# trinh-hoang-hiep/Collaborative-Filtering-Kafka

Measured on AMD Instinct MI355X. Metric: ALS ratings/sec per full iteration, k=64 Netflix-shape, 1/2/4/8 MI355X, higher is better.
Workload: dtype f32; 1 GPU; netflix-shape synthetic 480189 users x 17770 movies x 100000000 ratings, k=64, lambda=0.05, one step = one full ALS iteration; workload_name=netflix, n_movies=17770, nnz=100000000, nnz_this_rank=100000000, k=64, seed=2581, partitions=1, parallelism=id%1 shards + RCCL all-gather, rccl_world=1, exchange_world=1, rehearsal_gloo_one_gpu=False

## Files before the change

collaborative-filtering-kafka_amd/csrc/als_engine.cpp:

```cpp
#include <hip/hip_runtime.h>
#include <rccl/rccl.h>

#include <algorithm>
#include <chrono>
#include <cstdarg>
#include <cstdio>
#include <cstdlib>
#include <cstring>
#include <string>
#include <thread>
#include <vector>

#include "als.h"
#include "als_internal.h"

using cfk::Path;
using cfk::Task;

namespace {

thread_local std::string g_last_error;

int fail(int code, const char* fmt, ...) {
    char buf[1024];
// ... 8 lines not shown
#define HIP_TRY(expr)                                                                              \
    do {                                                                                           \
        hipError_t _e = (expr);                                                                    \
        if (_e != hipSuccess)                                                                      \
            return fail(ALS_ERR_DEVICE, "%s failed: %s (%s:%d)", #expr, hipGetErrorString(_e),     \
                        __FILE__, __LINE__);                                                       \
    } while (0)

struct Block {
    bool set = false;
    int64_t n_rows = 0, row_offset = 0, n_opp_rows = 0, nnz = 0, nnz_padded = 0;
    int32_t* d_col = nullptr;
    float* d_rat = nullptr;
    uint32_t* d_rat_pk = nullptr;
    int32_t* d_col_ps = nullptr;
    Task* d_tasks = nullptr;
    Task* d_reduce = nullptr;
    int32_t n_tasks = 0, n_reduce = 0, n_slots = 0;
    double* d_task_se = nullptr;
    std::vector<Task> h_tasks, h_reduce;
    Task* d_ctasks = nullptr;
    Task* d_creduce = nullptr;
    std::vector<int32_t> coff, croff;
    Task* d_dual[3] = {nullptr, nullptr, nullptr};
    int32_t n_dual[3] = {0, 0, 0};
    std::vector<Task> h_dual[3];
    Task* d_cdual[3] = {nullptr, nullptr, nullptr};
    std::vector<int32_t> cdoff[3];
    Task* d_sq_tasks = nullptr;
    int32_t n_sq = 0;
    cfk::BlockLayout layout;
    int64_t ilv_rows = 0, ilv_tasks = 0;
    int64_t rows_per_chunk = 0, chunk_stride = 0;
    int64_t factor_row(int64_t i) const {
        return rows_per_chunk > 0 ? row_offset + (i / rows_per_chunk) * chunk_stride + i % rows_per_chunk
                                  : row_offset + i;
    }
};

struct TimingRec {
    int side;
    hipEvent_t ev[3];
};

struct Factors {
    void* ptr = nullptr;
    int64_t n_rows = 0;
    bool owned = false;
};

struct Settings {
    cfk::PlanKnobs plan;
    bool gram_f32 = false;
    bool force_valu = false;
    float refine_min_pivot = 0.45f;
    bool dual_side = true;
    int64_t comm_timeout_ms = 120000;
    int32_t debug_flags = 0;
    uint32_t debug_gen_skew = 0;
    int32_t debug_extra_lds = 0;
    bool debug_fixed_gen = false;
};

}

namespace cfk_detail {
void set_last_error(const std::string& s) { g_last_error = s; }
}

struct als_engine {
    int device = 0;
    int k = 0, kp = 0;
    int precision = ALS_F32;
    Path path = Path::VALU;
    hipStream_t stream = nullptr;
    bool own_stream = false;
    Block blk[2];
    Factors fac[2];
    void* d_partials = nullptr;
    size_t partial_bytes = 0;
    int64_t generic_slabs = 0;
    void* d_split = nullptr;
    size_t split_bytes = 0;
    uint32_t* d_amax = nullptr;
    void* d_rec = nullptr;
    size_t rec_bytes = 0;
    void* h_stage = nullptr;
    size_t stage_bytes = 0;
    uint32_t* d_integrity = nullptr;
    int cu_count = 0;
    Settings cfg;
    uint32_t gen = 0;
    ncclComm_t comm = nullptr;
    int world = 1, rank = 0;
    hipStream_t comm_stream = nullptr;
    hipEvent_t solved = nullptr;
    hipEvent_t gathered[2] = {nullptr, nullptr};
    bool gather_pending[2] = {false, false};
    int last_gather_side = -1;
    int64_t last_gather_chunk = -1, last_gather_rows = 0;
    hipStream_t side_stream = nullptr;
    hipEvent_t fork = nullptr, join = nullptr;
    bool timing = false;
    std::vector<hipEvent_t> ev_pool;
    std::vector<TimingRec> pending;
    size_t elem() const { return precision == ALS_F64 ? 8 : 4; }
};

namespace {

int check_engine(const als_engine* e) {
    if (!e) return fail(ALS_ERR_INVALID_ARGUMENT, "engine is NULL");
    return ALS_OK;
}

int wait_gathers(als_engine* e, bool movie, bool user) {
    const bool want[2] = {movie, user};
    for (int s = 0; s < 2; ++s)
        if (want[s] && e->gather_pending[s]) {
            HIP_TRY(hipStreamWaitEvent(e->stream, e->gathered[s], 0));
            e->gather_pending[s] = false;
        }
    return ALS_OK;
}

int stream_wait(als_engine* e, hipStream_t s) {
    if (!e->comm || e->cfg.comm_timeout_ms <= 0) {
        HIP_TRY(hipStreamSynchronize(s));
        return ALS_OK;
    }
    const auto t0 = std::chrono::steady_clock::now();
    for (int spin = 0;; ++spin) {
        const hipError_t st = hipStreamQuery(s);
        if (st == hipSuccess) return ALS_OK;
        if (st != hipErrorNotReady) return fail(ALS_ERR_DEVICE, "stream wait: %s", hipGetErrorString(st));
        const int64_t ms =
            std::chrono::duration_cast<std::chrono::milliseconds>(std::chrono::steady_clock::now() - t0).count();
        if (ms > e->cfg.comm_timeout_ms) {
            (void)ncclCommAbort(e->comm);
            e->comm = nullptr;
            return fail(ALS_ERR_COMM,
                        "rank %d of %d: the engine's stream did not complete within %lld ms; the last RCCL all-gather "
                        "issued was side %s chunk %lld (%lld rows per shard); communicator aborted",
                        e->rank, e->world, (long long)e->cfg.comm_timeout_ms,
                        e->last_gather_side == ALS_SIDE_MOVIE ? "movie" : e->last_gather_side == ALS_SIDE_USER ? "user"
                                                                                                              : "none",
                        (long long)e->last_gather_chunk, (long long)e->last_gather_rows);
        }
        if (spin < 1000) std::this_thread::yield();
        else std::this_thread::sleep_for(std::chrono::microseconds(50));
    }
}

int sync_checked(als_engine* e) {
    if (int r = wait_gathers(e, true, true)) return r;
    if (int r = stream_wait(e, e->stream)) return r;
    uint32_t rec[cfk::INTEGRITY_WORDS];
    HIP_TRY(hipMemcpy(rec, e->d_integrity, sizeof(rec), hipMemcpyDeviceToHost));
    if (rec[0] != 0)
        return fail(ALS_ERR_INTEGRITY,
                    "%u REDUCE tasks found partial slots that failed their check (first: launch generation %u, slot "
                    "%u, row %u): partial sums its PARTIAL task's writes had not reached",
                    rec[0], rec[1], rec[2], rec[3]);
    return ALS_OK;
}
int check_side(int side) {
    if (side != ALS_SIDE_MOVIE && side != ALS_SIDE_USER)
// ... 36 lines not shown
#endif
    }
    if (const char* env = getenv("ALS_COMM_TIMEOUT_S")) c.comm_timeout_ms = (int64_t)(atof(env) * 1000.0);
#ifdef CFK_DEBUG_KNOBS
    if (const char* env = getenv("ALS_DEBUG_SKIP_SOLVE"))
        if (env[0] == '1') c.debug_flags |= cfk::SOLVE_FLAG_SKIP_SOLVE;
    if (const char* env = getenv("ALS_DEBUG_SKIP_REFINE"))
        if (env[0] == '1') c.debug_flags |= cfk::SOLVE_FLAG_SKIP_REFINE;
    if (const char* env = getenv("ALS_DEBUG_REDUCE_GEN_SKEW")) c.debug_gen_skew = (uint32_t)atoi(env);
    if (const char* env = getenv("ALS_DEBUG_FIXED_GEN")) c.debug_fixed_gen = env[0] == '1';
    if (const char* env = getenv("ALS_DEBUG_EXTRA_LDS")) c.debug_extra_lds = atoi(env);
    if (const char* env = getenv("ALS_ILV_CHUNK")) c.plan.ilv_chunk = std::max(32L, atol(env));
    if (const char* env = getenv("ALS_TASK_ORDER")) {
        if (std::strncmp(env, "stagger", 7) == 0) {
            c.plan.task_order = cfk::PlanKnobs::STAGGER;
            if (env[7] == ':') c.plan.stagger_window = std::max(1, atoi(env + 8));
        }
        if (std::strcmp(env, "random") == 0) c.plan.task_order = cfk::PlanKnobs::RANDOM;
    }
#endif
    return c;
}
}

extern "C" {

int als_abi_version(void) { return ALS_ABI_VERSION; }

int als_device_count(int* n) {
    if (!n) return fail(ALS_ERR_INVALID_ARGUMENT, "n is NULL");
    *n = 0;
    HIP_TRY(hipGetDeviceCount(n));
    return ALS_OK;
}
const char* als_last_error(void) { return g_last_error.c_str(); }

#define CFK_STR2(x) #x
#define CFK_STR(x) CFK_STR2(x)
const char* als_build_source_sha256(void) {
#ifdef CFK_SOURCE_SHA256
    return &CFK_STR(CFK_SOURCE_SHA256)[1];
#else
    return "";
#endif
}

int als_engine_create(int device, int num_features, int precision, als_engine** out) {
    if (!out) return fail(ALS_ERR_INVALID_ARGUMENT, "out is NULL");
    *out = nullptr;
    if (precision != ALS_F32 && precision != ALS_F64)
        return fail(ALS_ERR_INVALID_ARGUMENT, "precision must be ALS_F32 or ALS_F64");
    if (num_features < 1) return fail(ALS_ERR_INVALID_ARGUMENT, "num_features must be >= 1, got %d", num_features);
    if (num_features > 1024)
        return fail(ALS_ERR_UNSUPPORTED, "num_features=%d: this build supports 1..1024", num_features);
    const bool generic = num_features > (precision == ALS_F64 ? 64 : 128);
    int kp = num_features <= 16 ? 16 : num_features <= 32 ? 32 : num_features <= 64 ? 64 : 128;
    if (generic) kp = (num_features + 15) / 16 * 16;
    Path path = generic ? Path::GENERIC : (precision == ALS_F32 && num_features >= 32) ? Path::MFMA_SPLIT : Path::VALU;
    const Settings cfg = read_environment();
    if (path == Path::MFMA_SPLIT && cfg.gram_f32) path = Path::MFMA;
    if (cfg.force_valu && !generic) path = Path::VALU;
    if (!cfk::variant_available(precision, kp, path))
        return fail(ALS_ERR_UNSUPPORTED, "no kernel variant for precision=%d kp=%d", precision, kp);
    int ndev = 0;
    HIP_TRY(hipGetDeviceCount(&ndev));
    if (device < 0 || device >= ndev) return fail(ALS_ERR_INVALID_ARGUMENT, "device %d out of range (%d devices)", device, ndev);
    HIP_TRY(hipSetDevice(device));
    als_engine* e = new als_engine();
    e->device = device;
    e->k = num_features;
    e->kp = kp;
    e->precision = precision;
    e->path = path;
    e->cfg = cfg;
    hipError_t st = hipStreamCreateWithFlags(&e->stream, hipStreamNonBlocking);
    if (st != hipSuccess) {
        delete e;
        return fail(ALS_ERR_DEVICE, "hipStreamCreate: %s", hipGetErrorString(st));
    }
    e->own_stream = true;
    st = hipDeviceGetAttribute(&e->cu_count, hipDeviceAttributeMultiprocessorCount, device);
    if (st == hipSuccess) st = hipMalloc((void**)&e->d_integrity, cfk::INTEGRITY_WORDS * sizeof(uint32_t));
    if (st == hipSuccess) st = hipMemset(e->d_integrity, 0, cfk::INTEGRITY_WORDS * sizeof(uint32_t));
    if (st == hipSuccess) st = hipMalloc((void**)&e->d_amax, 2 * sizeof(uint32_t));
    if (st != hipSuccess) {
        (void)hipStreamDestroy(e->stream);
        (void)hipFree(e->d_integrity);
        (void)hipFree(e->d_amax);
        delete e;
        return fail(ALS_ERR_DEVICE, "integrity record: %s", hipGetErrorString(st));
    }
    *out = e;
    return ALS_OK;
}

int als_engine_destroy(als_engine* e) {
    if (!e) return ALS_OK;
    (void)hipSetDevice(e->device);
    (void)hipStreamSynchronize(e->stream);
    for (auto& b : e->blk) free_block(b);
    for (auto& f : e->fac)
        if (f.owned) (void)hipFree(f.ptr);
    (void)hipFree(e->d_partials);
    (void)hipFree(e->d_split);
    (void)hipFree(e->d_rec);
    (void)hipHostFree(e->h_stage);
    (void)hipFree(e->d_integrity);
    (void)hipFree(e->d_amax);
    for (auto& rec : e->pending)
        for (auto ev : rec.ev) (void)hipEventDestroy(ev);
    for (auto ev : e->ev_pool) (void)hipEventDestroy(ev);
    if (e->comm_stream) (void)hipStreamSynchronize(e->comm_stream);
    if (e->comm) (void)ncclCommDestroy(e->comm);
    if (e->comm_stream) (void)hipStreamDestroy(e->comm_stream);
    for (auto ev : {e->solved, e->gathered[0], e->gathered[1]})
        if (ev) (void)hipEventDestroy(ev);
    if (e->side_stream) {
        (void)hipStreamSynchronize(e->side_stream);
        (void)hipStreamDestroy(e->side_stream);
    }
    for (auto ev : {e->fork, e->join})
        if (ev) (void)hipEventDestroy(ev);
    if (e->own_stream) (void)hipStreamDestroy(e->stream);
    delete e;
    return ALS_OK;
}

int als_engine_set_stream(als_engine* e, void* hip_stream) {
    if (int r = check_engine(e)) return r;
    HIP_TRY(hipSetDevice(e->device));
    if (e->own_stream) {
        HIP_TRY(hipStreamSynchronize(e->stream));
        HIP_TRY(hipStreamDestroy(e->stream));
        e->own_stream = false;
        e->stream = nullptr;
    }
    if (hip_stream) {
        e->stream = (hipStream_t)hip_stream;
    } else {
        HIP_TRY(hipStreamCreateWithFlags(&e->stream, hipStreamNonBlocking));
        e->own_stream = true;
    }
    return ALS_OK;
}

int als_engine_use_default_stream(als_engine* e) {
    if (int r = check_engine(e)) return r;
    HIP_TRY(hipSetDevice(e->device));
    if (e->own_stream) {
        HIP_TRY(hipStreamSynchronize(e->stream));
        HIP_TRY(hipStreamDestroy(e->stream));
        e->own_stream = false;
    }
    e->stream = nullptr;
    return ALS_OK;
}

int als_factor_stride(const als_engine* e) { return e ? e->kp : 0; }

}

namespace {

int ensure_stage(als_engine* e) {
    constexpr size_t STAGE = 32u << 20;
    if (!e->h_stage) {
        HIP_TRY(hipHostMalloc(&e->h_stage, STAGE, hipHostMallocDefault));
        e->stage_bytes = STAGE;
    }
    return ALS_OK;
}

int check_block_shape(als_engine* e, int64_t n_rows, int64_t row_offset, int64_t n_opp_rows) {
    if (n_rows < 0 || row_offset < 0 || n_opp_rows < 0)
        return fail(ALS_ERR_INVALID_ARGUMENT, "negative size (n_rows=%lld row_offset=%lld n_opp_rows=%lld)",
                    (long long)n_rows, (long long)row_offset, (long long)n_opp_rows);
    if (n_rows > INT32_MAX) return fail(ALS_ERR_UNSUPPORTED, "n_rows exceeds 2^31-1");
    if (n_opp_rows >= INT32_MAX) return fail(ALS_ERR_UNSUPPORTED, "n_opp_rows must be < 2^31-1 (int32 column indices)");
    if ((n_opp_rows + 1) * (int64_t)e->kp * (int64_t)e->elem() > (int64_t)UINT32_MAX)
        return fail(ALS_ERR_UNSUPPORTED, "opposite factor matrix exceeds 4 GiB (32-bit gather offsets)");
    return ALS_OK;
}

inline int64_t padded(int64_t d) { return (d + cfk::BLOCK_ENTRIES - 1) / cfk::BLOCK_ENTRIES * cfk::BLOCK_ENTRIES; }

int upload_tasks(Task** dst, const std::vector<Task>& src) {
    if (*dst) {
        (void)hipFree(*dst);
        *dst = nullptr;
    }
    const size_t bytes = src.size() * sizeof(Task);
// ... 290 lines not shown
    const size_t row_bytes = (size_t)e->kp * es;
    if (int r = ensure_stage(e)) return r;
    const int64_t rows_per = (int64_t)(e->stage_bytes / row_bytes);
    for (int64_t r = 0; r < n_rows; r += rows_per) {
        const int64_t nr = std::min(rows_per, n_rows - r);
        HIP_TRY(cfk::launch_download((const char*)f.ptr + (size_t)(row0 + r) * row_bytes, e->h_stage,
                                     (size_t)nr * row_bytes, e->stream));
        HIP_TRY(hipStreamSynchronize(e->stream));
        const char* stage = (const char*)e->h_stage;
        char* dst = (char*)host_dst + (size_t)r * dst_ld * es;
        for (int64_t i = 0; i < nr; ++i)
            std::memcpy(dst + (size_t)i * dst_ld * es, stage + i * row_bytes, (size_t)e->k * es);
    }
    return ALS_OK;
}

namespace {

struct DualLaunch {
    const Task* t[3] = {nullptr, nullptr, nullptr};
    int32_t n[3] = {0, 0, 0};
};

int launch_half(als_engine* e, int side, float lambda, const Task* tasks, int32_t n_tasks, const Task* reduce,
                int32_t n_reduce, bool first_chunk, const DualLaunch& dl) {
    Block& b = e->blk[side];
    const Factors& self = e->fac[side];
    const Factors& opp = e->fac[1 - side];
    if (!self.ptr || !opp.ptr) return fail(ALS_ERR_STATE, "als_solve_half: factor matrices not allocated/bound");
    if (b.n_rows > 0 && b.factor_row(b.n_rows - 1) >= self.n_rows)
        return fail(ALS_ERR_STATE, "block rows (last at factor row %lld) exceed factor rows %lld",
                    (long long)b.factor_row(b.n_rows - 1), (long long)self.n_rows);
    if (b.n_opp_rows != opp.n_rows)
        return fail(ALS_ERR_STATE, "block was set for %lld opposite rows, the opposite factor matrix has %lld",
                    (long long)b.n_opp_rows, (long long)opp.n_rows);
    if (!(lambda >= 0.f)) return fail(ALS_ERR_INVALID_ARGUMENT, "lambda must be >= 0");
    HIP_TRY(hipSetDevice(e->device));
    if (int r = wait_gathers(e, side == ALS_SIDE_USER || first_chunk, side == ALS_SIDE_MOVIE || first_chunk)) return r;
    cfk::SolveArgs a{};
    a.tasks = tasks;
    a.n_tasks = n_tasks;
    a.k = e->k;
    a.col = b.d_col;
    a.rat = b.d_rat;
    a.opp = opp.ptr;
    a.out = self.ptr;
    a.row_offset = b.row_offset;
    a.rows_per_chunk = (int32_t)b.rows_per_chunk;
    a.chunk_stride = b.chunk_stride;
    a.partials = e->d_partials;
    a.scratch_slabs = e->generic_slabs;
    a.lambda = lambda;
    a.sentinel = (int32_t)b.n_opp_rows;
    a.flags = e->path == Path::VALU ? 0 : e->cfg.debug_flags;
    if (++e->gen == 0) e->gen = 1;
    a.gen = e->cfg.debug_fixed_gen ? 1u : e->gen;
    a.integrity = e->d_integrity;
    a.refine_min_pivot = e->cfg.refine_min_pivot;
    a.extra_lds = e->cfg.debug_extra_lds;
    TimingRec rec{side, {nullptr, nullptr, nullptr}};
    if (e->timing) {
        for (auto& ev : rec.ev) {
            if (!e->ev_pool.empty()) {
                ev = e->ev_pool.back();
                e->ev_pool.pop_back();
            } else {
                HIP_TRY(hipEventCreate(&ev));
            }
        }
        HIP_TRY(hipEventRecord(rec.ev[0], e->stream));
    }
    const bool any_dual = dl.n[0] > 0 || dl.n[1] > 0 || dl.n[2] > 0;
    const bool side_dual = any_dual && e->cfg.dual_side;
    if (side_dual) {
        if (!e->side_stream) {
            HIP_TRY(hipStreamCreateWithFlags(&e->side_stream, hipStreamNonBlocking));
            HIP_TRY(hipEventCreateWithFlags(&e->fork, hipEventDisableTiming));
            HIP_TRY(hipEventCreateWithFlags(&e->join, hipEventDisableTiming));
        }
        HIP_TRY(hipEventRecord(e->fork, e->stream));
    }
    if (b.layout.presplit) {
        if (first_chunk) {
            const int64_t n_floats = (b.n_opp_rows + 1) * (int64_t)e->kp;
            HIP_TRY(cfk::launch_absmax((const float*)opp.ptr, n_floats, e->kp, e->d_amax, e->stream));
            HIP_TRY(cfk::launch_presplit(e->kp, (const float*)opp.ptr, e->d_split, b.n_opp_rows + 1, e->d_amax,
                                         e->stream));
        }
        a.opp_split = e->d_split;
        a.rat_pk = b.d_rat_pk;
        a.rat_lo_off = b.nnz_padded / 2;
        a.col_ps = b.d_col_ps;
        a.amax = e->d_amax;
    }
    HIP_TRY(cfk::launch_solve(e->precision, e->kp, e->path, a, e->stream, b.layout.presplit, false));
    if (b.layout.presplit) {
        cfk::SolveArgs f = a;
        f.presplit_fallback = 1;
        f.grid_cap = 4 * e->cu_count;
        HIP_TRY(cfk::launch_solve(e->precision, e->kp, e->path, f, e->stream, false, false));
    }
    if (side_dual) HIP_TRY(hipStreamWaitEvent(e->side_stream, e->fork, 0));
    for (int c = 0; c < 3; ++c)
        if (dl.n[c] > 0) {
            cfk::SolveArgs d = a;
            d.tasks = dl.t[c];
            d.n_tasks = dl.n[c];
            HIP_TRY(cfk::launch_dual(e->kp, 2 * (c + 1), d, side_dual ? e->side_stream : e->stream));
        }
    if (side_dual) {
        HIP_TRY(hipEventRecord(e->join, e->side_stream));
        HIP_TRY(hipStreamWaitEvent(e->stream, e->join, 0));
    }
    if (e->timing) HIP_TRY(hipEventRecord(rec.ev[1], e->stream));
    if (n_reduce > 0) {
        a.tasks = reduce;
        a.n_tasks = n_reduce;
        a.gen += e->cfg.debug_gen_skew;
        HIP_TRY(cfk::launch_solve(e->precision, e->kp, e->path, a, e->stream, false, true));
    }
    if (e->timing) {
        HIP_TRY(hipEventRecord(rec.ev[2], e->stream));
        e->pending.push_back(rec);
    }
    return ALS_OK;
}

}

int als_solve_half(als_engine* e, int side, float lambda) {
    if (int r = check_engine(e)) return r;
    if (int r = check_side(side)) return r;
    Block& b = e->blk[side];
    if (!b.set) return fail(ALS_ERR_STATE, "als_solve_half: no block set for side %d", side);
    DualLaunch dl;
    for (int c = 0; c < 3; ++c) {
        dl.t[c] = b.d_dual[c];
        dl.n[c] = b.n_dual[c];
    }
    return launch_half(e, side, lambda, b.d_tasks, b.n_tasks, b.d_reduce, b.n_reduce, true, dl);
}

int als_set_chunks(als_engine* e, int side, int n_chunks, const int64_t* row_bounds) {
    if (int r = check_engine(e)) return r;
    if (int r = check_side(side)) return r;
    Block& b = e->blk[side];
    if (!b.set) return fail(ALS_ERR_STATE, "als_set_chunks: no block set for side %d", side);
    if (n_chunks < 1 || !row_bounds) return fail(ALS_ERR_INVALID_ARGUMENT, "n_chunks must be >= 1 with row_bounds");
    if (row_bounds[0] != 0 || row_bounds[n_chunks] != b.n_rows)
        return fail(ALS_ERR_INVALID_ARGUMENT, "row_bounds must run from 0 to n_rows (%lld)", (long long)b.n_rows);
    for (int c = 0; c < n_chunks; ++c)
        if (row_bounds[c + 1] < row_bounds[c]) return fail(ALS_ERR_INVALID_ARGUMENT, "row_bounds not monotone");
    std::vector<Task> ct, cr, cdl[3];
    cfk::partition_by_chunk(b.h_tasks, n_chunks, row_bounds, ct, b.coff);
    cfk::partition_by_chunk(b.h_reduce, n_chunks, row_bounds, cr, b.croff);
    for (int c = 0; c < 3; ++c) cfk::partition_by_chunk(b.h_dual[c], n_chunks, row_bounds, cdl[c], b.cdoff[c]);
    HIP_TRY(hipSetDevice(e->device));
    HIP_TRY(hipStreamSynchronize(e->stream));
    if (int r = upload_tasks(&b.d_ctasks, ct)) return r;
    if (int r = upload_tasks(&b.d_creduce, cr)) return r;
    for (int c = 0; c < 3; ++c)
        if (int r = upload_tasks(&b.d_cdual[c], cdl[c])) return r;
    return ALS_OK;
}

int als_solve_half_chunk(als_engine* e, int side, float lambda, int chunk) {
    if (int r = check_engine(e)) return r;
    if (int r = check_side(side)) return r;
    Block& b = e->blk[side];
    if (!b.set || b.coff.empty()) return fail(ALS_ERR_STATE, "als_solve_half_chunk: no chunks set for side %d", side);
    if (chunk < 0 || chunk + 1 >= (int)b.coff.size())
        return fail(ALS_ERR_INVALID_ARGUMENT, "chunk %d out of range (%d chunks)", chunk, (int)b.coff.size() - 1);
    DualLaunch dl;
    for (int c = 0; c < 3; ++c) {
        dl.t[c] = b.d_cdual[c] + b.cdoff[c][chunk];
        dl.n[c] = b.cdoff[c][chunk + 1] - b.cdoff[c][chunk];
// ... 438 lines not shown
```

collaborative-filtering-kafka_amd/csrc/als_internal.h:

```cpp
#pragma once
#include <cstdint>
#include <string>
#include <vector>

#include <hip/hip_runtime.h>

#include "als_plan.h"

namespace cfk {

struct SolveArgs {
    const Task* tasks;
    int32_t n_tasks;
    int32_t k;
    const int32_t* col;
    const float* rat;
    const void* opp;
    void* out;
    int64_t row_offset;
    void* partials;
    float lambda;
    int32_t sentinel;
    int32_t flags;
    const void* opp_split;
    uint32_t gen;
    uint32_t* integrity;
    float refine_min_pivot;
    const uint32_t* rat_pk;
    const int32_t* col_ps;
    int32_t rows_per_chunk;
    int64_t chunk_stride;
    int64_t rat_lo_off;
    const uint32_t* amax;
    int32_t presplit_fallback;
    int64_t scratch_slabs;
    int32_t grid_cap;
    int32_t extra_lds;
};
__host__ __device__ inline int64_t factor_row(int64_t row_offset, int32_t rows_per_chunk, int64_t chunk_stride,
                                              int32_t row) {
    if (rows_per_chunk <= 0) return row_offset + row;
    const int32_t q = row / rows_per_chunk;
    return row_offset + (int64_t)q * chunk_stride + (row - q * rows_per_chunk);
}
constexpr int INTEGRITY_WORDS = 4;
constexpr int32_t SOLVE_FLAG_SKIP_SOLVE = 1;
constexpr int32_t SOLVE_FLAG_SKIP_REFINE = 2;

struct SqErrArgs {
    const Task* tasks;
    int32_t n_tasks;
    const int32_t* col;
    const float* rat;
    const void* opp;
    const void* self;
    int64_t row_offset;
    double* task_se;
    int32_t sentinel;
    int32_t rows_per_chunk;
    int64_t chunk_stride;
};

struct GenericPlan {
    bool g_in_lds;
    int batch;
    int64_t lds_bytes;
    int64_t slab_elems;
};
GenericPlan generic_plan(int precision, int kp);
hipError_t launch_generic(int precision, int kp, const SolveArgs& a, hipStream_t s);

hipError_t launch_solve(int precision, int kp, Path path, const SolveArgs& a, hipStream_t s, bool presplit,
                        bool reduce);
hipError_t launch_permute_blocks(const int32_t* col, const float* rat, int32_t* col_out, float* rat_out,
                                 const int32_t* perm, int64_t n_blocks, hipStream_t s);
hipError_t launch_dual(int kp, int cd, const SolveArgs& a, hipStream_t s);
hipError_t launch_absmax(const float* src, int64_t n_floats, int kp, uint32_t* amax , hipStream_t s);
hipError_t launch_presplit(int kp, const float* src, void* dst, int64_t n_rows, const uint32_t* amax, hipStream_t s);
hipError_t launch_pack_cols_ps(const int32_t* col, int32_t* dst, int64_t n_entries, hipStream_t s);
hipError_t launch_pack_ratings(const float* rat, uint32_t* dst, int64_t n_pairs, hipStream_t s);
hipError_t launch_upload(const void* host_pinned, void* dst, size_t bytes, hipStream_t s);
hipError_t launch_download(const void* src, void* host_pinned, size_t bytes, hipStream_t s);
hipError_t launch_predict(int precision, const void* U, const void* M, int kp, int k, const int64_t* urows,
                          int64_t n_u, const int64_t* mrows, int64_t n_m, float* out, hipStream_t s);
hipError_t launch_recommend(int precision, const void* U, const void* M, int kp, int k, const int64_t* urows,
                            int64_t n_users, const int64_t* mrows, int64_t n_cand, int top_n,
                            const RecommendPlan& plan, const int64_t* excl_ptr, const int32_t* excl_idx,
                            float* part_score, int32_t* part_pos, float* out_score, int32_t* out_pos, hipStream_t s);
hipError_t launch_sq_error(int precision, int kp, const SqErrArgs& a, hipStream_t s);
int partial_words_per_lane(int precision, int kp, Path path);
int build_block_device(const int32_t* rows, const int32_t* cols, const int16_t* ratings, int64_t nnz, int64_t n_rows,
                       int64_t n_opp_rows, hipStream_t s, std::vector<int64_t>& deg, std::vector<int64_t>& begin,
                       int32_t** d_col, float** d_rat, std::string& err);
bool variant_available(int precision, int kp, Path path);

}
```

collaborative-filtering-kafka_amd/csrc/als_kernels.hip:

```cpp
#include <hip/hip_runtime.h>

#include <mutex>
#include <type_traits>
#include <utility>
#include <vector>

#include "als_internal.h"
#include "als_device.h"
#include "als_slots.h"
#include "als_lds_solve.h"
#include "als_mfma.h"
#include "als_tile_solve.h"
#include "als_gram.h"
#include "als_gram_presplit.h"
#include "als_generic.h"

namespace cfk {
namespace {

template <int KP>
constexpr int mfma_waves() { return WAVES; }

__global__ __launch_bounds__(256) void als_absmax(const u32x4* __restrict__ src, int64_t n4, int vpr,
                                                  uint32_t* __restrict__ out) {
    uint32_t m = 0, rmin = 0xffffffffu;
    const int64_t stride = (int64_t)gridDim.x * 256;
    for (int64_t i0 = (int64_t)blockIdx.x * 256 + (threadIdx.x & ~63); i0 < n4; i0 += stride) {
        const int64_t i = i0 + (threadIdx.x & 63);
        uint32_t v = 0;
        if (i < n4) {
            const u32x4 x = src[i] & 0x7fffffffu;
            v = max(max(x[0], x[1]), max(x[2], x[3]));
        }
        m = max(m, v);
        for (int o = 1; o < vpr; o <<= 1) v = max(v, (uint32_t)__shfl_xor((int)v, o));
        if (v != 0 && i < n4) rmin = min(rmin, v);
    }
#pragma unroll
    for (int o = 32; o > 0; o >>= 1) {
        m = max(m, (uint32_t)__shfl_xor((int)m, o));
        rmin = min(rmin, (uint32_t)__shfl_xor((int)rmin, o));
    }
    __shared__ uint32_t wm[4], wr[4];
    if ((threadIdx.x & 63) == 0) {
        wm[threadIdx.x >> 6] = m;
        wr[threadIdx.x >> 6] = rmin;
    }
    __syncthreads();
    if (threadIdx.x == 0) {
        m = max(max(wm[0], wm[1]), max(wm[2], wm[3]));
        rmin = min(min(wr[0], wr[1]), min(wr[2], wr[3]));
        if (m != 0) atomicMax(out, m);
        if (rmin != 0xffffffffu) atomicMax(out + 1, ~rmin);
    }
}
constexpr float PRESPLIT_RANGE = 65536.f;
__device__ __forceinline__ bool presplit_ok(const uint32_t* st) {
    const uint32_t mx = st[0], rc = st[1];
    if (mx >= 0x7f800000u) return false;
    if (rc == 0) return true;
    return __uint_as_float(mx) <= PRESPLIT_RANGE * __uint_as_float(~rc);
}

template <int KP>
__global__ __launch_bounds__(256) void als_presplit(const float* __restrict__ src, unsigned* __restrict__ dst,
                                                   int64_t n_threads, const uint32_t* __restrict__ amax) {
    constexpr int C = KP / 16;
    const int64_t t = (int64_t)blockIdx.x * 256 + threadIdx.x;
    if (t >= n_threads) return;
    const int sc = split_exp(*amax);
    const int64_t row = t / (2 * C);
    const int b = (int)(t % (2 * C)) >> 1, jh = (int)(t & 1);
    const float* s = src + row * KP + C * 8 * jh + b;
    u32x4 h, m;
#pragma unroll
    for (int i = 0; i < 4; ++i) {
        unsigned hh, mm;
        split2(ldexpf(s[C * (2 * i)], sc), ldexpf(s[C * (2 * i + 1)], sc), hh, mm);
        h[i] = hh;
        m[i] = mm;
    }
    unsigned* o = dst + row * (presplit_row_bytes(KP) / 4) + (16 * b + 8 * jh) / 2;
    *(u32x4*)o = h;
    *(u32x4*)(o + KP / 2) = m;
}
__global__ __launch_bounds__(256) void als_pack_cols_ps(const int32_t* __restrict__ col, int32_t* __restrict__ dst,
                                                       int64_t n) {
    const int64_t i = (int64_t)blockIdx.x * 256 + threadIdx.x;
    if (i >= n) return;
    const int w = (int)(i & 31), r = w >> 2, x = w & 3;
    const int k = 16 * (x >> 1) + 8 * (r >> 2) + 4 * (x & 1) + (r & 3);
    dst[i] = col[(i & ~(int64_t)31) + k];
}

template <int KP, int MINW, bool SPLIT, bool PRESPLIT = false, bool REDUCE = false, bool GRIDLOOP = false>
__global__ __launch_bounds__(64 * mfma_waves<KP>(), MINW) void als_solve_mfma(SolveArgs a) {
    constexpr int C = KP / 16;
    constexpr int NW = mfma_waves<KP>();
    using Acc = MfmaAcc<C>;
    __shared__ __attribute__((aligned(16))) float sbuf[NW][KP];
    constexpr bool TILES_LDS = tiles_in_lds<C>() && !(PRESPLIT && !REDUCE);
    constexpr int TL = TILES_LDS ? tile_lds_floats<C>() : 0;
    __shared__ __attribute__((aligned(16))) float tiles_lds[NW][TL > 0 ? TL : 1];
    (void)tiles_lds;
    constexpr int STAGE = (PRESPLIT && !REDUCE) ? 2 * C * 1024 : 16;
    __shared__ __attribute__((aligned(1024))) unsigned char stage_lds[NW][STAGE];
    (void)stage_lds;

    const int wave = threadIdx.x >> 6, lane = threadIdx.x & 63;
    if constexpr (!REDUCE && SPLIT) {
        if (PRESPLIT ? !presplit_ok(a.amax) : (a.presplit_fallback && presplit_ok(a.amax))) return;
    }
    auto task = [&](const int tid) {
        const Task tk = load_task(a.tasks + tid);
        float* buf = sbuf[wave];

        Acc acc;
#pragma unroll
        for (int p = 0; p < Acc::NT; ++p) acc.g[p] = f32x4{0.f, 0.f, 0.f, 0.f};
#pragma unroll
        for (int c = 0; c < C; ++c) acc.rhs[c] = 0.f;
        f32x4 E[C];
#pragma unroll
        for (int c = 0; c < C; ++c) E[c] = f32x4{0.f, 0.f, 0.f, 0.f};

        int ps_sc = 0;
        if constexpr (REDUCE) sum_partial_slots<C>(a, tk, acc, lane);
        else if constexpr (PRESPLIT) ps_sc = gram_presplit<KP>(a, tk, acc, E, stage_lds[uni(wave)], buf, lane);
        else if constexpr (SPLIT) gram_split<KP>(a, tk, acc, E, lane);
        else gram_f32<KP>(a, tk, acc, lane);

        if constexpr (SPLIT && !REDUCE) {
            if constexpr (PRESPLIT)
                fold_diag_lds<C>(acc, E, opaque(lane), stage_lds[uni(wave)]);
            else
                fold_diag<C>(acc, E, lane);
        }

        float u = 1.f;
        if constexpr (PRESPLIT && !REDUCE) u = rescale_presplit<C>(tk, acc, ps_sc);
        if (!REDUCE && tk.kind == TASK_PARTIAL) {
            store_partial<C>(a, tk, acc, lane);
            return;
        }
        if (a.flags & SOLVE_FLAG_SKIP_SOLVE) {
            float* out = (float*)a.out + factor_row(a.row_offset, a.rows_per_chunk, a.chunk_stride, tk.row) * (int64_t)KP;
            if (lane < 16) {
#pragma unroll
                for (int b = 0; b < C; ++b) out[C * lane + b] = acc.g[tile_index<C>(b, b)][0] + acc.rhs[b];
            }
            return;
        }
        if constexpr (TILES_LDS) {
            LdsTiles T{tiles_lds[wave] + 4 * lane};
            RegStore<C> A0;
#pragma unroll
            for (int p = 0; p < Acc::NT; ++p) T.put(p, acc.g[p]);
            solve_tiles<C>(T, A0, acc.rhs, buf, tk, a, lane);
        } else if constexpr (PRESPLIT && !REDUCE) {
            RegTiles<C> T{acc.g};
            RowResidual A0;
            solve_tiles<C>(T, A0, acc.rhs, buf, tk, a, lane, u);
        } else {
            RegTiles<C> T{acc.g};
            RegStore<C> A0;
            solve_tiles<C>(T, A0, acc.rhs, buf, tk, a, lane);
        }
// ... 332 lines not shown
}


bool variant_available(int precision, int kp, Path path) {
    if (path == Path::GENERIC) return kp % 16 == 0 && kp <= 1024;
    if (precision == 0) {
        if (path == Path::MFMA || path == Path::MFMA_SPLIT) return kp == 32 || kp == 64 || kp == 128;
        return kp == 16 || kp == 32 || kp == 64;
    }
    return path == Path::VALU && (kp == 16 || kp == 32 || kp == 64);
}

int partial_words_per_lane(int precision, int kp, Path path) {
    if (path == Path::GENERIC) return 0;
    if (path == Path::MFMA || path == Path::MFMA_SPLIT) {
        const int c = kp / 16;
        return (c * (c + 1) / 2) * 4 + c + 1;
    }
    return kp * kp / 64 + 1 + 1;
}

hipError_t launch_predict(int precision, const void* U, const void* M, int kp, int k, const int64_t* urows,
                          int64_t n_u, const int64_t* mrows, int64_t n_m, float* out, hipStream_t s) {
    if (n_u <= 0 || n_m <= 0) return hipSuccess;
    if (k > 128) {
        const int64_t cells = n_u * n_m;
        if ((cells + 255) / 256 > INT32_MAX) return hipErrorInvalidValue;
        const unsigned g = (unsigned)((cells + 255) / 256);
        if (precision == 0)
            als_predict_generic<float><<<g, 256, 0, s>>>((const float*)U, (const float*)M, kp, k, urows, n_u, mrows, n_m, out);
        else
            als_predict_generic<double><<<g, 256, 0, s>>>((const double*)U, (const double*)M, kp, k, urows, n_u, mrows,
                                                           n_m, out);
        return hipGetLastError();
    }
    if ((n_m + 15) / 16 > INT32_MAX || (n_u + 15) / 16 > 65535) return hipErrorInvalidValue;
    const dim3 grid((unsigned)((n_m + 15) / 16), (unsigned)((n_u + 15) / 16));
    if (precision == 0)
        als_predict_kernel<float><<<grid, 256, 0, s>>>((const float*)U, (const float*)M, kp, k, urows, n_u, mrows, n_m, out);
    else
        als_predict_kernel<double><<<grid, 256, 0, s>>>((const double*)U, (const double*)M, kp, k, urows, n_u, mrows, n_m,
                                                        out);
    return hipGetLastError();
}

__global__ __launch_bounds__(256) void copy16(const u32x4* __restrict__ src, u32x4* __restrict__ dst, int64_t n,
                                              int to_host) {
    const int64_t stride = (int64_t)gridDim.x * blockDim.x;
    for (int64_t i = (int64_t)blockIdx.x * blockDim.x + threadIdx.x; i < n; i += stride) {
        if (to_host) __builtin_nontemporal_store(src[i], dst + i);
        else dst[i] = __builtin_nontemporal_load(src + i);
    }
}

hipError_t launch_copy(const void* src, void* dst, size_t bytes, int to_host, hipStream_t s) {
    if (bytes == 0) return hipSuccess;
    if (bytes % 16 != 0) return hipErrorInvalidValue;
    const int64_t n = (int64_t)(bytes / 16);
    const int64_t blocks = std::min<int64_t>((n + 255) / 256, 4096);
    copy16<<<(unsigned)blocks, 256, 0, s>>>((const u32x4*)src, (u32x4*)dst, n, to_host);
    return hipGetLastError();
}
hipError_t launch_upload(const void* host_pinned, void* dst, size_t bytes, hipStream_t s) {
    return launch_copy(host_pinned, dst, bytes, 0, s);
}
hipError_t launch_download(const void* src, void* host_pinned, size_t bytes, hipStream_t s) {
    return launch_copy(src, host_pinned, bytes, 1, s);
}

__global__ __launch_bounds__(256) void als_pack_ratings(const float* __restrict__ rat, uint32_t* __restrict__ dst,
                                                        int64_t n_pairs) {
    const int64_t i = (int64_t)blockIdx.x * 256 + threadIdx.x;
    if (i >= n_pairs) return;
    unsigned h, m;
    split2(rat[2 * i], rat[2 * i + 1], h, m);
    dst[i] = h;
    dst[n_pairs + i] = m;
}
hipError_t launch_pack_ratings(const float* rat, uint32_t* dst, int64_t n_pairs, hipStream_t s) {
    if (n_pairs <= 0) return hipSuccess;
    als_pack_ratings<<<(unsigned)((n_pairs + 255) / 256), 256, 0, s>>>(rat, dst, n_pairs);
    return hipGetLastError();
}
hipError_t launch_absmax(const float* src, int64_t n_floats, int kp, uint32_t* amax, hipStream_t s) {
    hipError_t e = hipMemsetAsync(amax, 0, 2 * sizeof(uint32_t), s);
    if (e != hipSuccess || n_floats <= 0) return e;
    if (n_floats % kp || kp % 4 || kp / 4 > 64 || (kp / 4 & (kp / 4 - 1))) return hipErrorInvalidValue;
    const int64_t n4 = n_floats / 4;
    const int64_t blocks = std::max<int64_t>(1, std::min<int64_t>((n4 + 2047) / 2048, 512));
    als_absmax<<<(unsigned)blocks, 256, 0, s>>>((const u32x4*)src, n4, kp / 4, amax);
    return hipGetLastError();
}
hipError_t launch_presplit(int kp, const float* src, void* dst, int64_t n_rows, const uint32_t* amax, hipStream_t s) {
    const int64_t threads = n_rows * 2 * (kp / 16);
    if (threads <= 0) return hipSuccess;
    const unsigned grid = (unsigned)((threads + 255) / 256);
    if (kp == 64) als_presplit<64><<<grid, 256, 0, s>>>(src, (unsigned*)dst, threads, amax);
    else if (kp == 128) als_presplit<128><<<grid, 256, 0, s>>>(src, (unsigned*)dst, threads, amax);
    else return hipErrorInvalidValue;
    return hipGetLastError();
}
hipError_t launch_pack_cols_ps(const int32_t* col, int32_t* dst, int64_t n_entries, hipStream_t s) {
    if (n_entries <= 0) return hipSuccess;
    if (n_entries % BLOCK_ENTRIES) return hipErrorInvalidValue;
    als_pack_cols_ps<<<(unsigned)((n_entries + 255) / 256), 256, 0, s>>>(col, dst, n_entries);
    return hipGetLastError();
}

hipError_t launch_dual(int kp, int cd, const SolveArgs& a, hipStream_t s) {
    if (a.n_tasks <= 0) return hipSuccess;
    const unsigned grid = (unsigned)blocks_for(a.n_tasks);
    if (kp == 64 && cd == 2) als_solve_dual<64, 2><<<grid, 64 * WAVES, 0, s>>>(a);
    else if (kp == 128 && cd == 2) als_solve_dual<128, 2><<<grid, 64 * WAVES, 0, s>>>(a);
    else if (kp == 128 && cd == 4) als_solve_dual<128, 4><<<grid, 64 * WAVES, 0, s>>>(a);
    else if (kp == 128 && cd == 6) als_solve_dual<128, 6><<<grid, 64 * WAVES, 0, s>>>(a);
    else return hipErrorInvalidValue;
    return hipGetLastError();
}

hipError_t launch_solve(int precision, int kp, Path path, const SolveArgs& a, hipStream_t s, bool presplit,
                        bool reduce) {
    if (path == Path::GENERIC) return reduce ? hipErrorInvalidValue : launch_generic(precision, kp, a, s);
    if (precision == 0) {
        if (path == Path::MFMA) {
            if (kp == 32) return launch_solve_t<float, 32, Path::MFMA, 2>(a, s, reduce);
            if (kp == 64) return launch_solve_t<float, 64, Path::MFMA, 2>(a, s, reduce);
            if (kp == 128) return launch_solve_t<float, 128, Path::MFMA, 1>(a, s, reduce);
        } else if (path == Path::MFMA_SPLIT) {
            if (kp == 32) return launch_solve_t<float, 32, Path::MFMA_SPLIT, 2>(a, s, reduce);
            if (kp == 64 && presplit) return launch_solve_t<float, 64, Path::MFMA_SPLIT, PS64_WAVES, true>(a, s, reduce);
            if (kp == 64) return launch_solve_t<float, 64, Path::MFMA_SPLIT, 2>(a, s, reduce);
            if (kp == 128 && presplit) return launch_solve_t<float, 128, Path::MFMA_SPLIT, 1, true>(a, s, reduce);
            if (kp == 128) return launch_solve_t<float, 128, Path::MFMA_SPLIT, 1>(a, s, reduce);
        } else {
            if (kp == 16) return launch_solve_t<float, 16, Path::VALU>(a, s, reduce);
            if (kp == 32) return launch_solve_t<float, 32, Path::VALU>(a, s, reduce);
            if (kp == 64) return launch_solve_t<float, 64, Path::VALU>(a, s, reduce);
        }
    } else if (path == Path::VALU) {
        if (kp == 16) return launch_solve_t<double, 16, Path::VALU>(a, s, reduce);
        if (kp == 32) return launch_solve_t<double, 32, Path::VALU>(a, s, reduce);
        if (kp == 64) return launch_solve_t<double, 64, Path::VALU>(a, s, reduce);
    }
    return hipErrorInvalidValue;
}

GenericPlan generic_plan(int precision, int kp) {
    GenericPlan p{};
    const int64_t elem = precision == 0 ? 4 : 8;
    const int64_t ntri = (int64_t)kp * (kp + 1) / 2;
    const int64_t tri_b = ((ntri + 1) & ~(int64_t)1) * elem;
    const int64_t avail = 160 * 1024 - 1025 * elem - (precision == 0 ? 2 * 4 : (1024 + 64) * 8);
    const int64_t row_b = (int64_t)kp * elem;
    if (tri_b + 8 * row_b <= avail) {
        p.g_in_lds = true;
        p.batch = (int)std::min<int64_t>(64, (avail - tri_b) / row_b);
        p.lds_bytes = tri_b + p.batch * row_b;
        p.slab_elems = 0;
    } else {
        p.g_in_lds = false;
        p.batch = (int)std::max<int64_t>(1, std::min<int64_t>(64, (64 * 1024) / row_b));
        p.lds_bytes = p.batch * row_b;
        p.slab_elems = ntri + 1;
    }
    return p;
}

template <class T, bool L>
hipError_t launch_generic_t(const GenericPlan& p, int kp, const SolveArgs& a, hipStream_t s) {
    hipError_t e = ensure_dyn_lds((const void*)als_solve_generic<T, L>, (int)p.lds_bytes);
    if (e != hipSuccess) return e;
    int64_t grid = std::min<int64_t>(a.n_tasks, 4096);
    if (!L) grid = std::min<int64_t>(grid, a.scratch_slabs);
    if (grid <= 0) return hipErrorInvalidValue;
    als_solve_generic<T, L><<<(unsigned)grid, 256, (size_t)p.lds_bytes, s>>>(a, kp, p.batch, (T*)a.partials,
                                                                             p.slab_elems);
    return hipGetLastError();
}

hipError_t launch_generic(int precision, int kp, const SolveArgs& a, hipStream_t s) {
    if (a.n_tasks <= 0) return hipSuccess;
    if (kp > 1024 || kp % 16) return hipErrorInvalidValue;
    const GenericPlan p = generic_plan(precision, kp);
// ... 27 lines not shown
```

Before: 21.72 billion ratings/s.

## Fuse absmax scan with speculative presplit using predicted exponent from previous iteration

Replaces the separate memset, absmax reduction and presplit kernels with one fused scan kernel. The fused kernel presplits the opposite-side factors using the scale exponent predicted from the previous iteration of the same side while it also computes the max and min statistics. A small confirm kernel then recomputes the presplit only when the prediction was wrong. Double-buffered stat sets are reset in the confirm kernel, which removes the memset. This saves one full pass over the factor matrix per half-iteration when the exponent is stable, at the cost of a redundant pass when it changes.

```diff
diff --git a/collaborative-filtering-kafka_amd/csrc/als_engine.cpp b/collaborative-filtering-kafka_amd/csrc/als_engine.cpp
--- a/collaborative-filtering-kafka_amd/csrc/als_engine.cpp
+++ b/collaborative-filtering-kafka_amd/csrc/als_engine.cpp
@@ -114,7 +114,8 @@
     int64_t generic_slabs = 0;
     void* d_split = nullptr;
     size_t split_bytes = 0;
-    uint32_t* d_amax = nullptr;
+    uint32_t* d_prep = nullptr;
+    int prep_set = 0;
     void* d_rec = nullptr;
     size_t rec_bytes = 0;
     void* h_stage = nullptr;
@@ -317,11 +318,16 @@
     st = hipDeviceGetAttribute(&e->cu_count, hipDeviceAttributeMultiprocessorCount, device);
     if (st == hipSuccess) st = hipMalloc((void**)&e->d_integrity, cfk::INTEGRITY_WORDS * sizeof(uint32_t));
     if (st == hipSuccess) st = hipMemset(e->d_integrity, 0, cfk::INTEGRITY_WORDS * sizeof(uint32_t));
-    if (st == hipSuccess) st = hipMalloc((void**)&e->d_amax, 2 * sizeof(uint32_t));
+    {
+        uint32_t prep[2 * cfk::PREP_SET_WORDS + 2] = {};
+        prep[2 * cfk::PREP_SET_WORDS] = prep[2 * cfk::PREP_SET_WORDS + 1] = cfk::PREP_NO_EXP;
+        if (st == hipSuccess) st = hipMalloc((void**)&e->d_prep, sizeof(prep));
+        if (st == hipSuccess) st = hipMemcpy(e->d_prep, prep, sizeof(prep), hipMemcpyHostToDevice);
+    }
     if (st != hipSuccess) {
         (void)hipStreamDestroy(e->stream);
         (void)hipFree(e->d_integrity);
-        (void)hipFree(e->d_amax);
+        (void)hipFree(e->d_prep);
         delete e;
         return fail(ALS_ERR_DEVICE, "integrity record: %s", hipGetErrorString(st));
     }
@@ -341,7 +347,7 @@
     (void)hipFree(e->d_rec);
     (void)hipHostFree(e->h_stage);
     (void)hipFree(e->d_integrity);
-    (void)hipFree(e->d_amax);
+    (void)hipFree(e->d_prep);
     for (auto& rec : e->pending)
         for (auto ev : rec.ev) (void)hipEventDestroy(ev);
     for (auto ev : e->ev_pool) (void)hipEventDestroy(ev);
@@ -798,16 +804,17 @@
     }
     if (b.layout.presplit) {
         if (first_chunk) {
-            const int64_t n_floats = (b.n_opp_rows + 1) * (int64_t)e->kp;
-            HIP_TRY(cfk::launch_absmax((const float*)opp.ptr, n_floats, e->kp, e->d_amax, e->stream));
-            HIP_TRY(cfk::launch_presplit(e->kp, (const float*)opp.ptr, e->d_split, b.n_opp_rows + 1, e->d_amax,
-                                         e->stream));
+            e->prep_set ^= 1;
+            HIP_TRY(cfk::launch_presplit_prepare(e->kp, (const float*)opp.ptr, e->d_split, b.n_opp_rows + 1,
+                                                 e->d_prep + e->prep_set * cfk::PREP_SET_WORDS,
+                                                 e->d_prep + (e->prep_set ^ 1) * cfk::PREP_SET_WORDS,
+                                                 e->d_prep + 2 * cfk::PREP_SET_WORDS + side, e->cu_count, e->stream));
         }
         a.opp_split = e->d_split;
         a.rat_pk = b.d_rat_pk;
         a.rat_lo_off = b.nnz_padded / 2;
         a.col_ps = b.d_col_ps;
-        a.amax = e->d_amax;
+        a.amax = e->d_prep + e->prep_set * cfk::PREP_SET_WORDS;
     }
     HIP_TRY(cfk::launch_solve(e->precision, e->kp, e->path, a, e->stream, b.layout.presplit, false));
     if (b.layout.presplit) {
diff --git a/collaborative-filtering-kafka_amd/csrc/als_internal.h b/collaborative-filtering-kafka_amd/csrc/als_internal.h
--- a/collaborative-filtering-kafka_amd/csrc/als_internal.h
+++ b/collaborative-filtering-kafka_amd/csrc/als_internal.h
@@ -75,8 +75,11 @@
 hipError_t launch_permute_blocks(const int32_t* col, const float* rat, int32_t* col_out, float* rat_out,
                                  const int32_t* perm, int64_t n_blocks, hipStream_t s);
 hipError_t launch_dual(int kp, int cd, const SolveArgs& a, hipStream_t s);
-hipError_t launch_absmax(const float* src, int64_t n_floats, int kp, uint32_t* amax , hipStream_t s);
-hipError_t launch_presplit(int kp, const float* src, void* dst, int64_t n_rows, const uint32_t* amax, hipStream_t s);
+constexpr int PREP_SET_WORDS = 4;
+constexpr int PREP_EXP = 2;
+constexpr uint32_t PREP_NO_EXP = 0x7fffffffu;
+hipError_t launch_presplit_prepare(int kp, const float* src, void* dst, int64_t n_rows, uint32_t* set,
+                                   uint32_t* next_set, uint32_t* pred, int cu_count, hipStream_t s);
 hipError_t launch_pack_cols_ps(const int32_t* col, int32_t* dst, int64_t n_entries, hipStream_t s);
 hipError_t launch_pack_ratings(const float* rat, uint32_t* dst, int64_t n_pairs, hipStream_t s);
 hipError_t launch_upload(const void* host_pinned, void* dst, size_t bytes, hipStream_t s);
diff --git a/collaborative-filtering-kafka_amd/csrc/als_kernels.hip b/collaborative-filtering-kafka_amd/csrc/als_kernels.hip
--- a/collaborative-filtering-kafka_amd/csrc/als_kernels.hip
+++ b/collaborative-filtering-kafka_amd/csrc/als_kernels.hip
@@ -21,39 +21,6 @@
 template <int KP>
 constexpr int mfma_waves() { return WAVES; }
 
-__global__ __launch_bounds__(256) void als_absmax(const u32x4* __restrict__ src, int64_t n4, int vpr,
-                                                  uint32_t* __restrict__ out) {
-    uint32_t m = 0, rmin = 0xffffffffu;
-    const int64_t stride = (int64_t)gridDim.x * 256;
-    for (int64_t i0 = (int64_t)blockIdx.x * 256 + (threadIdx.x & ~63); i0 < n4; i0 += stride) {
-        const int64_t i = i0 + (threadIdx.x & 63);
-        uint32_t v = 0;
-        if (i < n4) {
-            const u32x4 x = src[i] & 0x7fffffffu;
-            v = max(max(x[0], x[1]), max(x[2], x[3]));
-        }
-        m = max(m, v);
-        for (int o = 1; o < vpr; o <<= 1) v = max(v, (uint32_t)__shfl_xor((int)v, o));
-        if (v != 0 && i < n4) rmin = min(rmin, v);
-    }
-#pragma unroll
-    for (int o = 32; o > 0; o >>= 1) {
-        m = max(m, (uint32_t)__shfl_xor((int)m, o));
-        rmin = min(rmin, (uint32_t)__shfl_xor((int)rmin, o));
-    }
-    __shared__ uint32_t wm[4], wr[4];
-    if ((threadIdx.x & 63) == 0) {
-        wm[threadIdx.x >> 6] = m;
-        wr[threadIdx.x >> 6] = rmin;
-    }
-    __syncthreads();
-    if (threadIdx.x == 0) {
-        m = max(max(wm[0], wm[1]), max(wm[2], wm[3]));
-        rmin = min(min(wr[0], wr[1]), min(wr[2], wr[3]));
-        if (m != 0) atomicMax(out, m);
-        if (rmin != 0xffffffffu) atomicMax(out + 1, ~rmin);
-    }
-}
 constexpr float PRESPLIT_RANGE = 65536.f;
 __device__ __forceinline__ bool presplit_ok(const uint32_t* st) {
     const uint32_t mx = st[0], rc = st[1];
@@ -63,26 +30,86 @@
 }
 
 template <int KP>
-__global__ __launch_bounds__(256) void als_presplit(const float* __restrict__ src, unsigned* __restrict__ dst,
-                                                   int64_t n_threads, const uint32_t* __restrict__ amax) {
+__device__ __forceinline__ uint32_t presplit_item(const float* __restrict__ src, unsigned* __restrict__ dst, int64_t t,
+                                                  int sc) {
     constexpr int C = KP / 16;
-    const int64_t t = (int64_t)blockIdx.x * 256 + threadIdx.x;
-    if (t >= n_threads) return;
-    const int sc = split_exp(*amax);
     const int64_t row = t / (2 * C);
     const int b = (int)(t % (2 * C)) >> 1, jh = (int)(t & 1);
     const float* s = src + row * KP + C * 8 * jh + b;
+    float x[8];
+#pragma unroll
+    for (int i = 0; i < 8; ++i) x[i] = s[C * i];
     u32x4 h, m;
+    uint32_t v = 0;
 #pragma unroll
     for (int i = 0; i < 4; ++i) {
         unsigned hh, mm;
-        split2(ldexpf(s[C * (2 * i)], sc), ldexpf(s[C * (2 * i + 1)], sc), hh, mm);
+        split2(ldexpf(x[2 * i], sc), ldexpf(x[2 * i + 1], sc), hh, mm);
         h[i] = hh;
         m[i] = mm;
+        v = max(v, max(__float_as_uint(x[2 * i]) & 0x7fffffffu, __float_as_uint(x[2 * i + 1]) & 0x7fffffffu));
     }
     unsigned* o = dst + row * (presplit_row_bytes(KP) / 4) + (16 * b + 8 * jh) / 2;
     *(u32x4*)o = h;
     *(u32x4*)(o + KP / 2) = m;
+    return v;
+}
+template <int KP>
+__global__ __launch_bounds__(1024) void als_presplit_scan(const float* __restrict__ src, unsigned* __restrict__ dst,
+                                                         int64_t n_items, const uint32_t* __restrict__ pred,
+                                                         uint32_t* __restrict__ set) {
+    const uint32_t p = *pred;
+    const int sc = p == PREP_NO_EXP ? 0 : (int)p;
+    uint32_t m = 0, rmin = 0xffffffffu;
+    const int64_t stride = (int64_t)gridDim.x * 1024;
+    for (int64_t t0 = (int64_t)blockIdx.x * 1024 + (threadIdx.x & ~63); t0 < n_items; t0 += stride) {
+        const int64_t t = t0 + (threadIdx.x & 63);
+        uint32_t v = t < n_items ? presplit_item<KP>(src, dst, t, sc) : 0;
+        m = max(m, v);
+#pragma unroll
+        for (int o = 1; o < 2 * (KP / 16); o <<= 1) v = max(v, (uint32_t)__shfl_xor((int)v, o));
+        if (v != 0 && t < n_items) rmin = min(rmin, v);
+    }
+#pragma unroll
+    for (int o = 32; o > 0; o >>= 1) {
+        m = max(m, (uint32_t)__shfl_xor((int)m, o));
+        rmin = min(rmin, (uint32_t)__shfl_xor((int)rmin, o));
+    }
+    __shared__ uint32_t wm[16], wr[16];
+    if ((threadIdx.x & 63) == 0) {
+        wm[threadIdx.x >> 6] = m;
+        wr[threadIdx.x >> 6] = rmin;
+    }
+    __syncthreads();
+    if (threadIdx.x < 64) {
+        m = threadIdx.x < 16 ? wm[threadIdx.x] : 0;
+        rmin = threadIdx.x < 16 ? wr[threadIdx.x] : 0xffffffffu;
+#pragma unroll
+        for (int o = 8; o > 0; o >>= 1) {
+            m = max(m, (uint32_t)__shfl_xor((int)m, o));
+            rmin = min(rmin, (uint32_t)__shfl_xor((int)rmin, o));
+        }
+        if (threadIdx.x == 0) {
+            if (m > __hip_atomic_load(set, __ATOMIC_RELAXED, __HIP_MEMORY_SCOPE_AGENT)) atomicMax(set, m);
+            if (~rmin > __hip_atomic_load(set + 1, __ATOMIC_RELAXED, __HIP_MEMORY_SCOPE_AGENT)) atomicMax(set + 1, ~rmin);
+            if (blockIdx.x == 0) set[PREP_EXP] = p;
+        }
+    }
+}
+template <int KP>
+__global__ __launch_bounds__(256) void als_presplit_confirm(const float* __restrict__ src, unsigned* __restrict__ dst,
+                                                           int64_t n_items, const uint32_t* __restrict__ set,
+                                                           uint32_t* __restrict__ next_set, uint32_t* __restrict__ pred) {
+    const int sc = split_exp(set[0]);
+    const bool right = set[PREP_EXP] == (uint32_t)sc;
+    if (blockIdx.x == 0 && threadIdx.x == 0) {
+        *pred = (uint32_t)sc;
+        next_set[0] = 0;
+        next_set[1] = 0;
+    }
+    if (right) return;
+    const int64_t stride = (int64_t)gridDim.x * 256;
+    for (int64_t t = (int64_t)blockIdx.x * 256 + threadIdx.x; t < n_items; t += stride) presplit_item<KP>(src, dst, t, sc);
 }
 __global__ __launch_bounds__(256) void als_pack_cols_ps(const int32_t* __restrict__ col, int32_t* __restrict__ dst,
                                                        int64_t n) {
@@ -581,23 +608,23 @@
     als_pack_ratings<<<(unsigned)((n_pairs + 255) / 256), 256, 0, s>>>(rat, dst, n_pairs);
     return hipGetLastError();
 }
-hipError_t launch_absmax(const float* src, int64_t n_floats, int kp, uint32_t* amax, hipStream_t s) {
-    hipError_t e = hipMemsetAsync(amax, 0, 2 * sizeof(uint32_t), s);
-    if (e != hipSuccess || n_floats <= 0) return e;
-    if (n_floats % kp || kp % 4 || kp / 4 > 64 || (kp / 4 & (kp / 4 - 1))) return hipErrorInvalidValue;
-    const int64_t n4 = n_floats / 4;
-    const int64_t blocks = std::max<int64_t>(1, std::min<int64_t>((n4 + 2047) / 2048, 512));
-    als_absmax<<<(unsigned)blocks, 256, 0, s>>>((const u32x4*)src, n4, kp / 4, amax);
-    return hipGetLastError();
-}
-hipError_t launch_presplit(int kp, const float* src, void* dst, int64_t n_rows, const uint32_t* amax, hipStream_t s) {
-    const int64_t threads = n_rows * 2 * (kp / 16);
-    if (threads <= 0) return hipSuccess;
-    const unsigned grid = (unsigned)((threads + 255) / 256);
-    if (kp == 64) als_presplit<64><<<grid, 256, 0, s>>>(src, (unsigned*)dst, threads, amax);
-    else if (kp == 128) als_presplit<128><<<grid, 256, 0, s>>>(src, (unsigned*)dst, threads, amax);
-    else return hipErrorInvalidValue;
-    return hipGetLastError();
+template <int KP>
+hipError_t launch_prepare_t(const float* src, void* dst, int64_t n_items, uint32_t* set, uint32_t* next_set,
+                            uint32_t* pred, int cu_count, hipStream_t s) {
+    const int cu = std::max(1, cu_count);
+    const unsigned gs = (unsigned)std::min<int64_t>((n_items + 1023) / 1024, 2 * cu);
+    als_presplit_scan<KP><<<gs, 1024, 0, s>>>(src, (unsigned*)dst, n_items, pred, set);
+    const unsigned gc = (unsigned)std::min<int64_t>((n_items + 255) / 256, 4 * cu);
+    als_presplit_confirm<KP><<<gc, 256, 0, s>>>(src, (unsigned*)dst, n_items, set, next_set, pred);
+    return hipGetLastError();
+}
+hipError_t launch_presplit_prepare(int kp, const float* src, void* dst, int64_t n_rows, uint32_t* set,
+                                   uint32_t* next_set, uint32_t* pred, int cu_count, hipStream_t s) {
+    if (n_rows <= 0) return hipErrorInvalidValue;
+    const int64_t n_items = n_rows * 2 * (kp / 16);
+    if (kp == 64) return launch_prepare_t<64>(src, dst, n_items, set, next_set, pred, cu_count, s);
+    if (kp == 128) return launch_prepare_t<128>(src, dst, n_items, set, next_set, pred, cu_count, s);
+    return hipErrorInvalidValue;
 }
 hipError_t launch_pack_cols_ps(const int32_t* col, int32_t* dst, int64_t n_entries, hipStream_t s) {
     if (n_entries <= 0) return hipSuccess;
```

After: 22.06 billion ratings/s (median of 6 runs). 1.02x the previous value.
